# nkkrnkl/category-agnostic-pose-estimation

Hardware: AMD Instinct MI355X
Metric: episodes/sec (1-shot, 256x256, 17kpt) training step (higher is better)
Workload: dtype f32 storage/accumulate, GEMMs as bf16x3 split (3 bf16 MFMAs per product); 1 GPU; configs[1]: 1-shot training step (fwd+loss+bwd+clip+AdamW at learning rate 0, dropout on), 256x256, 17 kpt, ResNet-50 + deformable transformer, 16 episodes x 2 queries per GPU; episodes_per_gpu=16, queries_per_episode=2, image_size=256, global_batch_episodes=16, parallelism=dp1, weights=random init (no checkpoint offline)

## Files before the change

### category-agnostic-pose-estimation_amd/hip/functional.py

```python
import contextlib
import ctypes
import os

import torch

from . import lib, ops


class Runtime:
    rng = None
    direct_grad = False
    use_side_stream = os.environ.get("CAPE_SIDE_STREAM", "1") == "1"
    side = None
    on_param_grad = []
    capture_keep = None

    pending = []
    side_dirty = False

    defer_wgrad = os.environ.get("CAPE_DEFER_WGRAD", "1") == "1"
    wgrad_group = int(os.environ.get("CAPE_WGRAD_GROUP", "12"))
    wq = {}
    wq_total = 0
    wq_notify = []
    _final_cb = False

    @classmethod
    def side_stream(cls):
        if cls.side is None:
            cls.side = torch.cuda.Stream()
            cls.side_raw = cls.side.cuda_stream
        return cls.side

    @classmethod
    def join(cls):
        cls.flush_wgrads()
        if cls.side is not None and cls.side_dirty:
            cls.side_dirty = False
            lib.call("cape_stream_join", ctypes.c_void_p(ops.raw_current_stream()), ctypes.c_void_p(cls.side_raw))
            if cls.capture_keep is None:
                cls.pending.clear()

    @classmethod
    def notify(cls, *params):
        if cls.wq_total or cls.wq_notify:
            cls.wq_notify.extend(p for p in params if p is not None)
            return
        for cb in cls.on_param_grad:
            for p in params:
                if p is not None:
                    cb(p)

    @classmethod
    def enqueue_wgrad(cls, desc, keep):
        M, N, K, b_mode = desc.M, desc.N, desc.K, desc.b_mode
        key = (ops.group_tile(M, N, K), b_mode, desc.precision)
        dst = [(desc.C, desc.C + 4 * ((M - 1) * desc.ldc + N))]
        if desc.colsum_out:
            dst.append((desc.colsum_out, desc.colsum_out + 4 * M))
        items = cls.wq.setdefault(key, [])
        if any(lo < e and s < hi for it in items for s, e in it[3] for lo, hi in dst):
            cls._launch_class(key)
        cls.wq[key].append((desc, keep, (M, N, K, 1, b_mode), dst))
        cls.wq_total += 1
        if not cls._final_cb:
            try:
                torch.autograd.Variable._execution_engine.queue_callback(cls.flush_wgrads)
                cls._final_cb = True
            except RuntimeError:
                cls.flush_wgrads()
                return
        if cls.wq_total >= cls.wgrad_group or len(cls.wq[key]) >= lib.GEMM_GROUP_MAX:
            cls._flush()

    @classmethod
    def _launch_class(cls, key):
        items = cls.wq.get(key)
        if not items:
            return
        cls.wq[key] = []
        cls.wq_total -= len(items)
        tile = key[0]
        shapes = [it[2] for it in items]
        for it, sk in zip(items, ops.plan_group_splits([sh[:3] for sh in shapes], tile)):
            it[0].split_k = sk
        with _Side([t for it in items for t in it[1]]):
            for i in range(0, len(items), lib.GEMM_GROUP_MAX):
                ops.gemm_group([it[0] for it in items[i:i + lib.GEMM_GROUP_MAX]], shapes[i:i + lib.GEMM_GROUP_MAX], tile)

    @classmethod
    def flush_wgrads(cls):
        cls._final_cb = False
        cls._flush()

    @classmethod
    def _flush(cls):
        for key in list(cls.wq):
            cls._launch_class(key)
        if cls.wq_notify:
            ps, cls.wq_notify = cls.wq_notify, []
            for cb in cls.on_param_grad:
                for p in ps:
                    cb(p)

    @classmethod
    def get_rng(cls, device):
        if cls.rng is None:
            cls.rng = ops.RngState(0x5EED, device)
        return cls.rng

    @classmethod
    def seed(cls, seed, device):
        cls.rng = ops.RngState(int(seed), device)


def capturing():
    return torch.cuda.is_available() and torch.cuda.is_current_stream_capturing()


def _c(t):
    return t if (t is None or t.is_contiguous()) else t.contiguous()


class _Side:

    def __init__(self, tensors):
        self.tensors = [t for t in tensors if t is not None]

    def __enter__(self):
        self.on, self.forked, self.prev = Runtime.use_side_stream, False, ops._side[0]
        if self.on:
            Runtime.side_stream()
            ops._side[0] = self._raw
        return self

    def _raw(self):
        if not self.forked:
            self.forked = True
            lib.call("cape_stream_fork", ctypes.c_void_p(ops.raw_current_stream()), ctypes.c_void_p(Runtime.side_raw))
            Runtime.side_dirty = True
        return Runtime.side_raw

    def __exit__(self, *a):
        if not self.on:
            return False
        ops._side[0] = self.prev
        (Runtime.capture_keep if Runtime.capture_keep is not None else Runtime.pending).extend(self.tensors)
        if len(Runtime.pending) > 8192:
            Runtime.join()
        return False


def _groupable(d):
    return (d.a_mode == 1 and d.accumulate and d.b_mode in (1, 3) and d.batch == 0 and d.mask_src is None and d.bias is None
            and d.A % 16 == 0 and d.B % 16 == 0 and d.lda % 4 == 0 and d.M % 4 == 0 and d.M >= 4 and d.N % 4 == 0 and d.N >= 4
            and (d.b_mode == 3 or d.ldb % 4 == 0) and max(d.lda, d.ldb, d.ldc) < (1 << 31))


_NO_SIDE = contextlib.nullcontext()


class _ParamGrads:

    def __init__(self, refs, needs=None):
        self.refs = refs
        self.needs = [r is not None and (needs is None or bool(needs[i])) for i, r in enumerate(refs)]
        views = [self._view(r) if n else None for r, n in zip(refs, self.needs)]
# ... 1174 lines not shown
```

### category-agnostic-pose-estimation_amd/hip/lib.py

```python
import ctypes
import os

import torch

from ctypes import POINTER, c_char_p, c_float, c_int, c_int32, c_int64, c_longlong, c_size_t, c_uint32, c_uint64, c_uint8, c_void_p

_HERE = os.path.dirname(os.path.abspath(__file__))
LIB_PATH = os.environ.get("CAPE_HIP_LIB", os.path.join(_HERE, "..", "csrc", "libcape_hip.so"))
LIB_PATH = os.path.abspath(LIB_PATH)

if not os.path.exists(LIB_PATH):
    raise ImportError(
        f"libcape_hip.so not found at {LIB_PATH}; build it with `python -c 'import __graft_entry__ as g; g.build()'` "
        "(or `make -C category-agnostic-pose-estimation_amd/csrc`).  There is no CPU fallback.")
try:
    _lib = ctypes.CDLL(LIB_PATH)
except OSError as e:
    raise ImportError(f"cannot load {LIB_PATH}: {e}") from e

_lib.cape_last_error.restype = c_char_p
_lib.cape_abi_version.restype = c_int


class GemmDesc(ctypes.Structure):
# ... 7 lines not shown
        ("rng_state", c_void_p), ("rng_stream", c_uint32), ("colsum_out", c_void_p), ("precision", c_int),
        ("B_packed", c_void_p),
        ("mask_src", c_void_p), ("ldm", c_longlong), ("mask_scale", c_float),
        ("batch", c_int), ("batch_div", c_int), ("sA0", c_longlong), ("sA1", c_longlong), ("sB0", c_longlong), ("sB1", c_longlong),
        ("sC0", c_longlong), ("sC1", c_longlong),
        ("res_cols", c_int), ("sBias0", c_longlong), ("sBias1", c_longlong),
        ("cPadX", c_int), ("cKHp", c_int), ("cKWp", c_int), ("cTapH0", c_int), ("cTapHS", c_int), ("cTapW0", c_int), ("cTapWS", c_int),
    ]


class PackItem(ctypes.Structure):
    _fields_ = [("B", c_void_p), ("out", c_void_p), ("ldb", c_longlong), ("N", c_int), ("K", c_int), ("b_mode", c_int), ("pad", c_int)]


class DecodeLinearDesc(ctypes.Structure):
    _fields_ = [
        ("N", c_int), ("K", c_int), ("Nout", c_int),
        ("X", c_void_p), ("ldx", c_longlong), ("in_gamma", c_void_p), ("in_beta", c_void_p), ("in_add", c_void_p), ("ld_add", c_longlong),
        ("W", c_void_p), ("ldw", c_longlong), ("bias", c_void_p),
        ("X2", c_void_p), ("ldx2", c_longlong), ("K2", c_int), ("W2", c_void_p), ("ldw2", c_longlong), ("n2", c_int),
        ("R", c_void_p), ("ldr", c_longlong), ("res_gamma", c_void_p), ("res_beta", c_void_p),
        ("relu", c_int), ("nseg", c_int), ("seg", c_int), ("out", c_void_p * 3), ("ldo", c_longlong * 3),
    ]


class DecodeTailDesc(ctypes.Structure):
    _fields_ = [
        ("N", c_int), ("L", c_int),
        ("P4", c_void_p), ("ldp", c_longlong), ("g3", c_void_p), ("b3", c_void_p),
        ("W1", c_void_p), ("B1", c_void_p), ("W2", c_void_p), ("B2", c_void_p), ("W3", c_void_p), ("B3", c_void_p),
        ("ref", c_void_p),
        ("Wc", c_void_p), ("Bc", c_void_p), ("ncls", c_int),
        ("Wp", c_void_p), ("Bp", c_void_p), ("gp", c_void_p), ("bp", c_void_p),
        ("dim_t", c_void_p), ("vr", c_void_p),
        ("ref_out", c_void_p), ("ld_ref", c_longlong),
        ("qpos_out", c_void_p), ("refin_out", c_void_p),
        ("cls_out", c_void_p), ("ld_cls", c_longlong),
        ("hs_out", c_void_p), ("ld_hs", c_longlong),
    ]


class AugItem(ctypes.Structure):
    _fields_ = [("src", c_void_p), ("aug", c_void_p), ("out", c_void_p), ("stat", c_void_p), ("h", c_int), ("w", c_int),
                ("M", c_float * 6), ("color_on", c_int), ("order", c_int * 4),
                ("bright", c_float), ("contrast", c_float), ("sat", c_float), ("hue", c_float),
                ("mode", c_int), ("noise_std", c_float), ("seed", c_uint32), ("blur_k", c_int), ("blur_w", c_float * 49)]


DECODE_MAX_LAYERS = 8
GEMM_GROUP_MAX = 32
SUMSQ_PARTS = 256


class DecodeLayerDesc(ctypes.Structure):
    _fields_ = [(n, c_void_p) for n in (
        "w_qkv", "b_qkv", "w_qin", "k_cache", "v_cache", "w_o", "b_o", "ln2_g", "ln2_b",
        "w_sq", "b_sq", "sup_k", "sup_v", "sup_mask", "w_so", "b_so", "lns_g", "lns_b",
        "w_off", "b_off", "value", "w_mo", "b_mo", "ln1_g", "ln1_b",
        "w1", "b1", "w2", "b2", "ln3_g", "ln3_b", "m1w", "m1b", "m2w", "m2b", "m3w", "m3b")]


class DecodeStepDesc(ctypes.Structure):
    _fields_ = [
        ("N", c_int), ("n_layers", c_int), ("step", c_int), ("T", c_int), ("P", c_int), ("S", c_int), ("L", c_int),
        ("n_points", c_int), ("ncls", c_int), ("ffn_dim", c_int),
        ("shapes", c_int * 8), ("level_start", c_int * 4),
        ("emb", c_void_p), ("qpos0", c_void_p), ("refin0", c_void_p), ("ref0", c_void_p), ("vr", c_void_p), ("dim_t", c_void_p),
        ("class_w", c_void_p), ("class_b", c_void_p),
        ("pos_w", c_void_p), ("pos_b", c_void_p), ("pos_gamma", c_void_p), ("pos_beta", c_void_p),
        ("out_logits", c_void_p), ("ld_logits", c_longlong),
        ("out_coords", c_void_p), ("ld_coords", c_longlong),
        ("out_hs", c_void_p), ("ld_hs", c_longlong),
        ("layers", DecodeLayerDesc * DECODE_MAX_LAYERS),
    ]


P, I, LL, F, U32 = c_void_p, c_int, c_longlong, c_float, c_uint32
_SIGS = {
    "cape_rng_advance": [P, P],
    "cape_stream_fork": [P, P],
    "cape_stream_join": [P, P],
    "cape_gemm_f32": [POINTER(GemmDesc), P],
    "cape_gemm_group_f32": [POINTER(GemmDesc), I, I, P],
    "cape_pack_weights": [P, I, I, P],
    "cape_colsum_f32": [P, LL, I, LL, I, I, P, I, P],
    "cape_add_layernorm_fwd": [P, P, P, P, P, P, P, P, P, I, I, F, P, U32, P],
    "cape_add_layernorm_bwd": [P, P, P, P, P, P, P, P, P, P, P, I, I, F, P, U32, P],
    "cape_groupnorm_fwd": [P, P, P, P, LL, P, P, I, I, I, I, P, c_size_t, P],
    "cape_groupnorm_bwd": [P, LL, P, P, P, P, P, P, P, I, I, I, I, P, c_size_t, P],
    "cape_msda_fwd": [P, P, P, P, P, P, I, I, I, I, I, P],
    "cape_msda_bwd": [P, P, P, P, P, P, P, P, P, I, I, I, I, I, P],
    "cape_msda_bwd_ex": [P, P, P, P, P, P, P, P, P, I, I, I, I, I, I, P],
    "cape_msda_bwd_atomic": [P, P, P, P, P, P, P, P, P, I, I, I, I, I, P],
    "cape_attn_fwd": [P, P, P, P, P, LL, LL, LL, LL, LL, LL, LL, LL, I, I, I, I, F, I, I, P, F, P, U32, P],
    "cape_attn_bwd": [P, P, P, P, P, P, P, P, P, LL, LL, LL, LL, LL, LL, LL, LL, I, I, I, I, F, I, I, P, F, P, U32, P],
    "cape_flash_attn_fwd": [P, P, P, P, P, LL, LL, LL, LL, LL, LL, LL, LL, I, I, I, I, F, I, I, P, F, P, U32, P],
    "cape_flash_attn_bwd": [P, P, P, P, P, P, P, P, P, P, LL, LL, LL, LL, LL, LL, LL, LL, I, I, I, I, F, I, I, P, F, P, U32, P],
    "cape_attn_softmax_fwd": [P, P, P, I, I, I, I, F, I, I, P, F, P, U32, P],
    "cape_attn_softmax_bwd": [P, P, I, I, I, I, F, F, P, U32, P],
    "cape_add_f32": [P, P, P, LL, P],
    "cape_level_embed_add": [P, P, P, P, I, I, I, I, P],
    "cape_add_n_f32": [POINTER(c_void_p), I, P, LL, P],
    "cape_add_n_rows_f32": [POINTER(c_void_p), POINTER(c_longlong), I, P, LL, LL, I, P],
    "cape_augment_batch": [P, I, I, I, P, P, P],
    "cape_gelu_f32": [P, P, LL, P],
    "cape_support_masks": [P, P, P, I, I, I, P],
    "cape_interleave2x2_f32": [POINTER(c_void_p), P, P, I, I, I, I, P],
    "cape_gelu_bwd_f32": [P, P, P, LL, P],
    "cape_scale_residual_bwd_f32": [P, P, P, P, P, LL, I, P],
    "cape_scale_residual_f32": [P, P, P, P, LL, I, P],
    "cape_nchw_to_nhwc": [P, P, I, I, I, I, I, P],
    "cape_bn_fold": [P, P, P, P, F, P, P, I, P],
    "cape_maxpool3x3s2_nhwc": [P, P, I, I, I, I, P],
    "cape_bn_relu_bwd": [P, P, P, P, P, LL, I, I, P],
    "cape_affine_act_f32": [P, P, P, P, LL, I, I, P],
    "cape_relu_drop_bwd": [P, P, P, LL, F, P],
    "cape_pos_sine_level": [P, P, P, P, LL, I, I, I, I, P],
    "cape_token_embed_fwd": [P, P, P, P, P, P, P, P, P, P, LL, I, I, P],
    "cape_token_embed_bwd": [P, P, P, P, P, P, P, P, P, P, LL, I, I, I, P],
    "cape_query_sine_fwd": [P, P, P, LL, P],
    "cape_query_sine_bwd": [P, P, P, P, I, LL, P],
    "cape_refine_fwd": [P, P, P, LL, P],
    "cape_refine_bwd": [P, P, P, P, P, I, LL, P],
    "cape_sigmoid_fwd": [P, P, LL, P],
    "cape_sigmoid_bwd": [P, P, P, I, LL, P],
    "cape_ref_scale_fwd": [P, P, P, LL, I, I, P],
    "cape_ref_scale_bwd": [P, P, P, I, LL, I, I, P],
    "cape_support_embed_fwd": [P, P, P, P, P, P, P, I, I, I, P],
    "cape_support_embed_bwd": [P, P, P, P, P, I, I, I, P],
    "cape_adjacency": [P, P, P, P, I, I, P],
    "cape_gcn_aggregate_fwd": [P, P, P, I, I, I, P],
    "cape_gcn_aggregate_bwd": [P, P, P, P, I, I, I, P],
    "cape_zero_rows": [P, P, LL, I, P],
    "cape_legacy_coord_embed_fwd": [P, P, P, P, I, I, P],
    "cape_legacy_coord_embed_bwd": [P, P, P, P, P, P, P, I, I, P],
    "cape_support_edge_info_fwd": [P, P, P, P, LL, P, P, P, I, I, I, P],
    "cape_support_edge_info_bwd": [P, LL, P, P, P, I, I, P],
    "cape_pe_dropout_fwd": [P, P, P, I, I, I, F, P, U32, P],
    "cape_pe_dropout_bwd": [P, P, LL, F, P, U32, P],
    "cape_loss_fwd_bwd": [P, P, P, P, P, P, F, F, F, P, P, P, P, I, LL, P],
    "cape_sumsq": [P, LL, P, P],
    "cape_adamw_step": [P, P, P, P, LL, F, F, F, F, F, F, P, I, P, P, P],
    "cape_step_increment": [P, P],
    "cape_decode_next_tokens": [P, P, P, P, P, P, I, I, I, I, I, I, P],
    "cape_decode_advance": [P, LL, P, LL, P, P, P, I, I, I, I, I, I, I, P, I, I, P, P, P],
    "cape_decode_linear": [POINTER(DecodeLinearDesc), P],
    "cape_decode_tail": [POINTER(DecodeTailDesc), P],
    "cape_decode_step": [POINTER(DecodeStepDesc), P],
}
EXPORTS = ["cape_last_error", "cape_abi_version", "cape_groupnorm_workspace_bytes", "cape_packed_weight_bytes"] + list(_SIGS)
_lib.cape_packed_weight_bytes.argtypes = [I, I]
_lib.cape_packed_weight_bytes.restype = c_size_t
_lib.cape_groupnorm_workspace_bytes.argtypes = [I, I, I]
_lib.cape_groupnorm_workspace_bytes.restype = c_size_t

for _name, _args in _SIGS.items():
    _fn = getattr(_lib, _name)
    _fn.argtypes = _args
    _fn.restype = c_int


def last_error() -> str:
    return _lib.cape_last_error().decode()


def abi_version() -> int:
    return _lib.cape_abi_version()


def call(name, *args):
    rc = getattr(_lib, name)(*args)
    if rc != 0:
        raise RuntimeError(f"{name} failed: {last_error()}")


def raw():
    return _lib
```

### category-agnostic-pose-estimation_amd/hip/ops.py

```python
import ctypes
import math
import os
import weakref

import torch

from . import lib

_F32 = torch.float32


_raw_stream = getattr(torch._C, "_cuda_getCurrentRawStream", None)
_raw_device = getattr(torch._C, "_cuda_getDevice", None)


_side = [None]


def raw_current_stream():
    if _raw_stream is not None and _raw_device is not None:
        return _raw_stream(_raw_device())
    return torch.cuda.current_stream().cuda_stream


# ... 216 lines not shown
            (d.cPadX, d.cKHp, d.cKWp, d.cTapH0, d.cTapHS, d.cTapW0, d.cTapWS) = conv_sub
            assert a_mode == 3 and b_mode == 2 and _avail(B) >= d.cO * d.cKHp * d.cKWp * d.cC
            assert _avail(A) >= d.cN * d.cOH * d.cOW * d.cO and _avail(C) >= d.cN * d.cH * d.cW * d.cC
    d.scale = scale.data_ptr() if scale is not None else None
    d.bias = bias.data_ptr() if bias is not None else None
    d.residual = residual.data_ptr() if residual is not None else None
    d.ldr = ldr if ldr is not None else N
    d.res_cols = int(res_cols)
    d.relu, d.accumulate, d.split_k = int(relu), int(accumulate), int(split_k)
    d.dropout_p = float(dropout_p)
    d.rng_state = rng.t.data_ptr() if (rng is not None and dropout_p > 0) else None
    d.rng_stream = rng_stream
    d.precision = GEMM_PRECISION
    if (packed is None and PackedWeights.enabled and GEMM_PRECISION >= 1 and a_mode == 0 and b_mode in (0, 1) and batch is None
            and split_k == 1 and K in (64, 128, 256) and M > 64 and 32 <= N <= _PACK_MAX_N):
        packed = PackedWeights.lookup(B, N, K, d.ldb, b_mode)
    if packed is not None and GEMM_PRECISION >= 1:
        assert packed.dtype == torch.int16 and packed.is_cuda and packed.numel() * 2 >= lib.raw().cape_packed_weight_bytes(N, K)
        d.B_packed = packed.data_ptr()
    if mask_src is not None:
        _chk(mask_src, "gemm.mask_src")
        assert mask_src.numel() == M * N and split_k == 1
        d.mask_src, d.ldm, d.mask_scale = mask_src.data_ptr(), N, float(mask_scale)
    if colsum_out is not None:
        _chk(colsum_out, "gemm.colsum_out", contiguous=False)
        assert a_mode == 1 and _avail(colsum_out) >= M
        d.colsum_out = colsum_out.data_ptr()
    if batch is not None:
        cnt, div, sA0, sA1, sB0, sB1, sC0, sC1 = batch
        assert cnt >= 1 and div >= 1 and cnt % div == 0
        d.batch, d.batch_div = cnt, div
        d.sA0, d.sA1, d.sB0, d.sB1, d.sC0, d.sC1 = sA0, sA1, sB0, sB1, sC0, sC1
        if bias_strides is not None:
            d.sBias0, d.sBias1 = bias_strides
            assert bias is not None and _avail(bias) >= (cnt // div - 1) * d.sBias0 + (div - 1) * d.sBias1 + N
        last0, last1 = cnt // div - 1, div - 1
        offA, offB, offC = last0 * sA0 + last1 * sA1, last0 * sB0 + last1 * sB1, last0 * sC0 + last1 * sC1
    else:
        offA = offB = offC = 0
    if a_mode == 0 and M > 0:
        assert _avail(A) >= offA + (M - 1) * d.lda + K, "gemm: A too small"
    if a_mode == 1 and K > 0:
        assert _avail(A) >= offA + (K - 1) * d.lda + M, "gemm: A^T too small"
    if b_mode == 0 and N > 0:
        assert _avail(B) >= offB + (N - 1) * d.ldb + K, "gemm: B too small"
    if b_mode == 1 and K > 0:
        assert _avail(B) >= offB + (K - 1) * d.ldb + N, "gemm: B too small"
    if M > 0:
        assert _avail(C) >= offC + (M - 1) * d.ldc + N, "gemm: C too small"
    if residual is not None:
        assert res_cols % 32 == 0 and 0 <= res_cols <= N
        assert _avail(residual) >= (M - 1) * d.ldr + (res_cols or N), "gemm: residual too small"
    if bias is not None:
        assert _avail(bias) >= N
    if scale is not None:
        assert scale.numel() >= N
    return d, (A, B, C, colsum_out)


def launch_gemm(d):
    if GemmProfiler.enabled:
        e0, e1 = torch.cuda.Event(enable_timing=True), torch.cuda.Event(enable_timing=True)
        st = _stream()
        ext = torch.cuda.ExternalStream(st.value) if _side[0] is not None else None
        e0.record(ext)
        lib.call("cape_gemm_f32", ctypes.byref(d), st)
        e1.record(ext)
        M, N, K, nb = d.M, d.N, d.K, max(d.batch, 1)
        GemmProfiler.records.append((e0, e1, 2.0 * M * N * K * nb, (M, N, K, d.a_mode, d.b_mode, d.split_k, nb),
                                     GemmProfiler.alg_bytes(M, N, K, nb), 1))
        return
    lib.call("cape_gemm_f32", ctypes.byref(d), _stream())


_AUTO_SPLIT_NN = os.environ.get("CAPE_AUTO_SPLIT_NN", "1") == "1" and os.environ.get("CAPE_DETERMINISTIC", "0") != "1"
_PACK_MAX_N = int(os.environ.get("CAPE_PACK_MAX_N", "1000000"))
_GROUP_BIG_MN = int(os.environ.get("CAPE_GROUP_BIG_MN", str(64 * 1024)))


def group_tile(M, N, K):
    return 128 if (M >= 128 and N >= 128 and M * N >= _GROUP_BIG_MN and K >= 4096) else 64


def plan_group_splits(shapes, tile):
    target = 1024 if tile == 64 else 512
    tiles = [((M + tile - 1) // tile) * ((N + tile - 1) // tile) for M, N, K in shapes]
    kt = [(K + 31) // 32 for M, N, K in shapes]
    work = sum(t * k for t, k in zip(tiles, kt))
    per_block = max(8.0, work / float(target))
    out = []
    for k in kt:
        s = int(max(1, min(round(k / per_block), k // 8 if k >= 16 else 1, 64)))
        if s >= 8:
            s = s // 8 * 8
        out.append(s)
    return out


def gemm_group(descs, shapes, tile):
    n = len(descs)
    assert 1 <= n <= lib.GEMM_GROUP_MAX
    arr = (lib.GemmDesc * n)(*descs)
    if GemmProfiler.enabled:
        e0, e1 = torch.cuda.Event(enable_timing=True), torch.cuda.Event(enable_timing=True)
        st = _stream()
        ext = torch.cuda.ExternalStream(st.value) if _side[0] is not None else None
        e0.record(ext)
        lib.call("cape_gemm_group_f32", arr, n, tile, st)
        e1.record(ext)
        fl = sum(2.0 * M * N * K for M, N, K, _, _ in shapes)
        by = sum(GemmProfiler.alg_bytes(M, N, K) for M, N, K, _, _ in shapes)
        GemmProfiler.records.append((e0, e1, fl, ("group", tile, shapes[0][4], n), by, n))
        return
    lib.call("cape_gemm_group_f32", arr, n, tile, _stream())


def colsum(X, M, N, out, ldx=None, accumulate=True, nbatch=1, batch_stride=0):
    _chk(X, "colsum.X", contiguous=False)
    _chk(out, "colsum.out", contiguous=False)
    ldx = N if ldx is None else ldx
    assert M == 0 or _avail(X) >= (nbatch - 1) * batch_stride + (M - 1) * ldx + N
    assert _avail(out) >= N
    lib.call("cape_colsum_f32", _p(X), ldx, nbatch, batch_stride, M, N, _p(out), int(accumulate), _stream())


def add_layernorm_fwd(x, y, gamma, beta, pos=None, dropout_p=0.0, rng=None, rng_stream=0):
    C = x.shape[-1]
    rows = x.numel() // C
    for t, n in ((x, "x"), (y, "y"), (gamma, "gamma"), (beta, "beta"), (pos, "pos")):
        _chk(t, "ln." + n)
    if y is not None:
        assert y.shape == x.shape
    if pos is not None:
        assert pos.numel() == x.numel()
    out = torch.empty_like(x)
    mean = torch.empty(rows, dtype=_F32, device=x.device)
    rstd = torch.empty(rows, dtype=_F32, device=x.device)
    out_pos = torch.empty_like(x) if pos is not None else None
    lib.call("cape_add_layernorm_fwd", _p(x), _p(y), _p(gamma), _p(beta), _p(out), _p(mean), _p(rstd), _p(pos),
             _p(out_pos), rows, C, float(dropout_p), rng.ptr if (rng is not None and dropout_p > 0) else None,
             rng_stream, _stream())
    return out, mean, rstd, out_pos


def add_layernorm_bwd(d_out, d_out_pos, x, y, gamma, mean, rstd, dgamma, dbeta, dropout_p=0.0, rng=None, rng_stream=0):
    C = x.shape[-1]
    rows = x.numel() // C
    for t, n in ((d_out, "d_out"), (d_out_pos, "d_out_pos"), (x, "x"), (y, "y"), (dgamma, "dgamma"), (dbeta, "dbeta")):
        _chk(t, "ln_bwd." + n)
    d_x = torch.empty_like(x)
    d_y = torch.empty_like(x) if (y is not None and dropout_p > 0) else None
    lib.call("cape_add_layernorm_bwd", _p(d_out), _p(d_out_pos), _p(x), _p(y), _p(gamma), _p(mean), _p(rstd), _p(d_x),
             _p(d_y), _p(dgamma), _p(dbeta), rows, C, float(dropout_p),
             rng.ptr if (rng is not None and dropout_p > 0) else None, rng_stream, _stream())
    return d_x, (d_y if d_y is not None else d_x)


def _gn_workspace(N, C, G, device):
    nbytes = lib.raw().cape_groupnorm_workspace_bytes(N, C, G)
    return torch.empty((nbytes + 7) // 8, dtype=torch.float64, device=device), nbytes


def groupnorm_fwd(x, gamma, beta, out, out_image_stride, N, HW, C, G=32):
    for t, n in ((x, "x"), (gamma, "gamma"), (beta, "beta")):
        _chk(t, "gn." + n)
    _chk(out, "gn.out", contiguous=False)
    assert x.numel() == N * HW * C
    mean = torch.empty(N * G, dtype=_F32, device=x.device)
    rstd = torch.empty(N * G, dtype=_F32, device=x.device)
    ws, nbytes = _gn_workspace(N, C, G, x.device)
    lib.call("cape_groupnorm_fwd", _p(x), _p(gamma), _p(beta), _p(out), out_image_stride, _p(mean), _p(rstd), N, HW, C, G,
             _p(ws), nbytes, _stream())
    return mean, rstd


def groupnorm_bwd(d_out, d_out_image_stride, x, gamma, mean, rstd, dgamma, dbeta, N, HW, C, G=32):
    _chk(d_out, "gn_bwd.d_out", contiguous=False)
    d_x = torch.empty_like(x)
    ws, nbytes = _gn_workspace(N, C, G, x.device)
    lib.call("cape_groupnorm_bwd", _p(d_out), d_out_image_stride, _p(x), _p(gamma), _p(mean), _p(rstd), _p(d_x),
             _p(dgamma), _p(dbeta), N, HW, C, G, _p(ws), nbytes, _stream())
    return d_x


class LevelGeometry:

    def __init__(self, shapes):
        self.shapes = [(int(h), int(w)) for h, w in shapes]
        self.L = len(self.shapes)
        starts, s = [], 0
        for h, w in self.shapes:
            starts.append(s)
            s += h * w
        self.S = s
        self.starts = starts
        self._shapes_c = (ctypes.c_int * (2 * self.L))(*[v for hw in self.shapes for v in hw])
        self._starts_c = (ctypes.c_int * self.L)(*starts)
# ... 798 lines not shown
```

### include/cape_hip.h

```cpp
#ifndef CAPE_HIP_H
#define CAPE_HIP_H

#include <stddef.h>
#include <stdint.h>

#ifdef __cplusplus
extern "C" {
#endif

typedef void* cape_stream_t;

const char* cape_last_error(void);
int cape_abi_version(void);

int cape_rng_advance(uint64_t* rng_state, cape_stream_t stream);

int cape_stream_fork(cape_stream_t main_stream, cape_stream_t side_stream);
int cape_stream_join(cape_stream_t main_stream, cape_stream_t side_stream);

typedef struct {
  int M, N, K;
  int a_mode, b_mode;
  const float* A; long long lda;
  const float* B; long long ldb;
  float* C; long long ldc;
  int cN, cH, cW, cC, cKH, cKW, cStride, cPad, cOH, cOW, cO;
  const float* scale;
  const float* bias;
  const float* residual;
  long long ldr;
  int relu;
  int accumulate;
  int split_k;
  float dropout_p;
  const uint64_t* rng_state;
  uint32_t rng_stream;
  float* colsum_out;
  int precision;
  const uint16_t* B_packed;
  const float* mask_src; long long ldm; float mask_scale;
  int batch, batch_div; long long sA0, sA1, sB0, sB1, sC0, sC1;
  int res_cols; long long sBias0, sBias1;
  int cPadX, cKHp, cKWp, cTapH0, cTapHS, cTapW0, cTapWS;
} cape_gemm_desc;

int cape_gemm_f32(const cape_gemm_desc* d, cape_stream_t stream);

#define CAPE_GEMM_GROUP_MAX 32
int cape_gemm_group_f32(const cape_gemm_desc* descs, int n, int tile, cape_stream_t stream);

typedef struct { const float* B; uint16_t* out; long long ldb; int N, K, b_mode, pad; } cape_pack_item;
size_t cape_packed_weight_bytes(int N, int K);
int cape_pack_weights(const cape_pack_item* items_dev, int n_items, int max_blocks_per_item, cape_stream_t stream);

int cape_colsum_f32(const float* X, long long ldx, int nbatch, long long batch_stride, int M, int N, float* out,
                    int accumulate, cape_stream_t stream);

typedef struct {
  int N, K, Nout;
  const float* X; long long ldx; const float* in_gamma; const float* in_beta; const float* in_add; long long ld_add;
  const float* W; long long ldw; const float* bias;
  const float* X2; long long ldx2; int K2; const float* W2; long long ldw2; int n2;
  const float* R; long long ldr; const float* res_gamma; const float* res_beta;
  int relu;
  int nseg, seg; float* out[3]; long long ldo[3];
} cape_decode_linear_desc;
int cape_decode_linear(const cape_decode_linear_desc* d, cape_stream_t stream);

typedef struct {
  int N, L;
  const float* P4; long long ldp; const float* g3; const float* b3;
  const float* W1; const float* B1; const float* W2; const float* B2; const float* W3; const float* B3;
  const float* ref;
  const float* Wc; const float* Bc; int ncls;
  const float* Wp; const float* Bp; const float* gp; const float* bp;
  const float* dim_t; const float* vr;
  float* ref_out; long long ld_ref;
  float* qpos_out; float* refin_out;
  float* cls_out; long long ld_cls;
  float* hs_out; long long ld_hs;
} cape_decode_tail_desc;
int cape_decode_tail(const cape_decode_tail_desc* d, cape_stream_t stream);

#define CAPE_DECODE_MAX_LAYERS 8
typedef struct {
  const float *w_qkv, *b_qkv;
  const float* w_qin;
  float *k_cache, *v_cache;
  const float *w_o, *b_o, *ln2_g, *ln2_b;
  const float *w_sq, *b_sq;
  const float *sup_k, *sup_v;
  const unsigned char* sup_mask;
  const float *w_so, *b_so, *lns_g, *lns_b;
  const float *w_off, *b_off;
  const float* value;
  const float *w_mo, *b_mo, *ln1_g, *ln1_b;
  const float *w1, *b1, *w2, *b2;
  const float *ln3_g, *ln3_b;
  const float *m1w, *m1b, *m2w, *m2b, *m3w, *m3b;
} cape_decode_layer_desc;
typedef struct {
  int N, n_layers, step, T, P, S, L, n_points, ncls, ffn_dim;
  int shapes[8];
  int level_start[4];
  const float* emb;
  const float* qpos0;
  const float* refin0;
  const float* ref0;
  const float* vr;
  const float* dim_t;
  const float *class_w, *class_b;
  const float *pos_w, *pos_b, *pos_gamma, *pos_beta;
  float* out_logits; long long ld_logits;
  float* out_coords; long long ld_coords;
  float* out_hs; long long ld_hs;
  cape_decode_layer_desc layers[CAPE_DECODE_MAX_LAYERS];
} cape_decode_step_desc;
int cape_decode_step(const cape_decode_step_desc* d, cape_stream_t stream);

int cape_add_layernorm_fwd(const float* x, const float* y, const float* gamma, const float* beta,
                           float* out, float* mean, float* rstd, const float* pos, float* out_pos,
                           int rows, int C, float dropout_p, const uint64_t* rng_state, uint32_t rng_stream,
                           cape_stream_t stream);
int cape_add_layernorm_bwd(const float* d_out, const float* d_out_pos, const float* x, const float* y,
                           const float* gamma, const float* mean, const float* rstd,
                           float* d_x, float* d_y, float* dgamma, float* dbeta,
                           int rows, int C, float dropout_p, const uint64_t* rng_state, uint32_t rng_stream,
                           cape_stream_t stream);

size_t cape_groupnorm_workspace_bytes(int N, int C, int G);
int cape_groupnorm_fwd(const float* x, const float* gamma, const float* beta, float* out,
                       long long out_image_stride, float* mean, float* rstd,
                       int N, int HW, int C, int G, void* workspace, size_t workspace_bytes, cape_stream_t stream);
// ... 161 lines not shown
```

Measured before the change: 650.4 episodes/s.

## Add ordered split-K weight-gradient grouped GEMM with workspace reduction and larger tiles

Adds a dedicated grouped weight-gradient GEMM kernel with 256x128 tiles. Split-K partials are written to a workspace slab, and the last-arriving block, chosen by an atomic ticket counter, sums them in a fixed order and accumulates the result into C, with the bias colsum fused in. This replaces the previous grouped path for tile-128 dense bf16x3 and single-bf16 weight gradients. The split planner targets fewer blocks sized for the new tile. It adds a persistent workspace and counter buffer, allocated with a device sync outside capture, plus extra global traffic for the partial slabs. Reduction order becomes deterministic.

```diff
diff --git a/category-agnostic-pose-estimation_amd/csrc/gemm_wgrad.hip b/category-agnostic-pose-estimation_amd/csrc/gemm_wgrad.hip
--- /dev/null
+++ b/category-agnostic-pose-estimation_amd/csrc/gemm_wgrad.hip
@@ -0,0 +1,377 @@
+#include "gemm_common.h"
+
+namespace {
+
+constexpr int WG_MAX = CAPE_GEMM_GROUP_MAX;
+constexpr int WBM = 256, WBN = 128, WBK = 16;
+constexpr int TILE_F = WBM * WBN;
+constexpr int SLAB_F = TILE_F + WBM;
+constexpr int PLANE_B = WBK * 128 * 2;
+constexpr int BUF_B = 6 * PLANE_B;
+
+struct WgItem {
+  const float* A; const float* B; float* C; float* colsum_out;
+  float* ws; int* ctr;
+  int M, N, K, nsplit;
+  int lda, ldb, ldc, tilesN;
+  int ntiles, per, pad0, pad1;
+};
+
+struct WgArgs {
+  int n, single;
+  int bstart[WG_MAX + 1];
+  int pad;
+  WgItem it[WG_MAX];
+};
+static_assert(sizeof(WgArgs) <= 4096, "the item table travels as kernel arguments");
+
+template <bool KFULL>
+__global__ void __launch_bounds__(256, 2) gemm_wgrad_kernel(const WgArgs g) {
+  __shared__ __attribute__((aligned(16))) char lds[2 * BUF_B];
+
+  int bid = blockIdx.x;
+  int it_i = 0;
+  while (it_i + 1 < g.n && bid >= g.bstart[it_i + 1]) ++it_i;
+  const WgItem& q = g.it[it_i];
+  bid -= g.bstart[it_i];
+  const int ntiles = q.ntiles, nsplit = q.nsplit;
+  if (bid >= ntiles * nsplit) return;
+
+  int tile, split;
+  {
+    const int xcd = bid & 7, loc = bid >> 3;
+    if (nsplit > 1 && (nsplit & 7) == 0) {
+      split = xcd + 8 * (loc / ntiles);
+      tile = loc % ntiles;
+    } else if (nsplit > 1) {
+      split = bid / ntiles;
+      tile = bid - split * ntiles;
+    } else {
+      const int qq = ntiles >> 3, r = ntiles & 7;
+      tile = (xcd < r ? xcd * (qq + 1) : r * (qq + 1) + (xcd - r) * qq) + loc;
+      split = 0;
+    }
+  }
+  const int tm = tile / q.tilesN, tn = tile - tm * q.tilesN;
+  const int m0 = tm * WBM, n0 = tn * WBN;
+  const int M = q.M, N = q.N, K = q.K;
+
+  const int kb = split * q.per * BK;
+  const int ke = min(K, kb + q.per * BK);
+  const int nk = (ke - kb + WBK - 1) / WBK;
+
+  const int t = threadIdx.x;
+  const int lane = t & 63;
+  const int wave = t >> 6;
+  const int wm = wave >> 1, wn = wave & 1;
+
+  const int mc = t & 31, k0 = t >> 5;
+  const float* a_src0 = q.A + min(m0 + 4 * mc, M - 4);
+  const float* a_src1 = q.A + min(m0 + 128 + 4 * mc, M - 4);
+  const float* b_src = q.B + min(n0 + 4 * mc, N - 4);
+  const long long lda = q.lda, ldb = q.ldb;
+  const int st_off0 = tr_off<128>(2 * k0, mc >> 1) + 8 * (mc & 1);
+  const int st_off1 = tr_off<128>(2 * k0 + 1, mc >> 1) + 8 * (mc & 1);
+
+  float4 ra[2][2], rb[2];
+  auto load_tile = [&](int kt) {
+#pragma unroll
+    for (int j = 0; j < 2; ++j) {
+      const int k = kb + kt * WBK + 2 * k0 + j;
+      const bool kin = KFULL || k < K;
+      const long long kr = kin ? k : 0;
+      const float4 v0 = *reinterpret_cast<const float4*>(a_src0 + kr * lda);
+      const float4 v1 = *reinterpret_cast<const float4*>(a_src1 + kr * lda);
+      const float4 w = *reinterpret_cast<const float4*>(b_src + kr * ldb);
+      ra[0][j] = kin ? v0 : zero4();
+      ra[1][j] = kin ? v1 : zero4();
+      rb[j] = kin ? w : zero4();
+    }
+  };
+
+  const bool do_colsum = q.colsum_out != nullptr && tn == 0;
+  float4 csum[2] = {zero4(), zero4()};
+
+  auto store_tile = [&](int buf) {
+    char* base = lds + buf * BUF_B;
+    if (do_colsum) {
+#pragma unroll
+      for (int im = 0; im < 2; ++im)
+#pragma unroll
+        for (int j = 0; j < 2; ++j) { csum[im].x += ra[im][j].x; csum[im].y += ra[im][j].y; csum[im].z += ra[im][j].z; csum[im].w += ra[im][j].w; }
+    }
+#pragma unroll
+    for (int j = 0; j < 2; ++j) {
+      const int o = j ? st_off1 : st_off0;
+#pragma unroll
+      for (int im = 0; im < 2; ++im) {
+        unsigned h0, l0, h1, l1;
+        split2(ra[im][j].x, ra[im][j].y, h0, l0);
+        split2(ra[im][j].z, ra[im][j].w, h1, l1);
+        *reinterpret_cast<uint2*>(base + (2 * im) * PLANE_B + o) = make_uint2(h0, h1);
+        *reinterpret_cast<uint2*>(base + (2 * im + 1) * PLANE_B + o) = make_uint2(l0, l1);
+      }
+      unsigned h0, l0, h1, l1;
+      split2(rb[j].x, rb[j].y, h0, l0);
+      split2(rb[j].z, rb[j].w, h1, l1);
+      *reinterpret_cast<uint2*>(base + 4 * PLANE_B + o) = make_uint2(h0, h1);
+      *reinterpret_cast<uint2*>(base + 5 * PLANE_B + o) = make_uint2(l0, l1);
+    }
+  };
+
+  f32x16 acc[4][2];
+#pragma unroll
+  for (int i = 0; i < 4; ++i)
+#pragma unroll
+    for (int j = 0; j < 2; ++j)
+#pragma unroll
+      for (int r = 0; r < 16; ++r) acc[i][j][r] = 0.f;
+
+  const int tr_h = lane >> 5, tr_c = (lane >> 4) & 1, tr_q = (lane >> 2) & 3, tr_p = lane & 3;
+  const int fr_row = 8 * tr_h + tr_q, fr_chunk = 2 * tr_c + (tr_p >> 1), fr_sub = 8 * (tr_p & 1);
+  int a_fr[4], b_fr[2];
+#pragma unroll
+  for (int i = 0; i < 4; ++i) a_fr[i] = (2 * wm) * PLANE_B + tr_off<128>(fr_row, 4 * i + fr_chunk) + fr_sub;
+#pragma unroll
+  for (int j = 0; j < 2; ++j) b_fr[j] = 4 * PLANE_B + tr_off<128>(fr_row, 8 * wn + 4 * j + fr_chunk) + fr_sub;
+
+  auto compute_tile = [&](int buf) {
+    const char* base = lds + buf * BUF_B;
+    bf16x8 ahi[4], alo[4], bhi[2], blo[2];
+#pragma unroll
+    for (int i = 0; i < 4; ++i) {
+      ahi[i] = tr_read8(base + a_fr[i], 4 * 128 * 2);
+      alo[i] = tr_read8(base + a_fr[i] + PLANE_B, 4 * 128 * 2);
+    }
+#pragma unroll
+    for (int j = 0; j < 2; ++j) {
+      bhi[j] = tr_read8(base + b_fr[j], 4 * 128 * 2);
+      blo[j] = tr_read8(base + b_fr[j] + PLANE_B, 4 * 128 * 2);
+    }
+#pragma unroll
+    for (int i = 0; i < 4; ++i)
+#pragma unroll
+      for (int j = 0; j < 2; ++j) {
+        if (!g.single) {
+          acc[i][j] = __builtin_amdgcn_mfma_f32_32x32x16_bf16(alo[i], bhi[j], acc[i][j], 0, 0, 0);
+          acc[i][j] = __builtin_amdgcn_mfma_f32_32x32x16_bf16(ahi[i], blo[j], acc[i][j], 0, 0, 0);
+        }
+        acc[i][j] = __builtin_amdgcn_mfma_f32_32x32x16_bf16(ahi[i], bhi[j], acc[i][j], 0, 0, 0);
+      }
+  };
+
+  load_tile(0);
+  store_tile(0);
+  if (nk > 1) load_tile(1);
+  __syncthreads();
+  int cur = 0;
+  for (int kt = 0; kt < nk; ++kt) {
+    compute_tile(cur);
+    if (kt + 1 < nk) store_tile(cur ^ 1);
+    __syncthreads();
+    if (kt + 2 < nk) load_tile(kt + 2);
+    cur ^= 1;
+  }
+
+  float4 bias4 = zero4();
+  if (do_colsum) {
+    float4* red = reinterpret_cast<float4*>(lds);
+    red[t] = csum[0];
+    red[256 + t] = csum[1];
+    __syncthreads();
+    if (t < 64) {
+      const float4* src = red + 256 * (t >> 5) + mc;
+#pragma unroll
+      for (int i = 0; i < 8; ++i) { const float4 u = src[32 * i]; bias4.x += u.x; bias4.y += u.y; bias4.z += u.z; bias4.w += u.w; }
+    }
+    __syncthreads();
+  }
+
+  if (nsplit > 1) {
+    float* slab0 = q.ws + (long long)tile * nsplit * SLAB_F;
+    float4* mine = reinterpret_cast<float4*>(slab0 + (long long)split * SLAB_F) + wave * 2048 + lane;
+#pragma unroll
+    for (int i = 0; i < 4; ++i)
+#pragma unroll
+      for (int j = 0; j < 2; ++j)
+#pragma unroll
+        for (int r4 = 0; r4 < 4; ++r4)
+          mine[((2 * i + j) * 4 + r4) * 64] = make_float4(acc[i][j][4 * r4], acc[i][j][4 * r4 + 1], acc[i][j][4 * r4 + 2], acc[i][j][4 * r4 + 3]);
+    if (do_colsum && t < 64) *reinterpret_cast<float4*>(slab0 + (long long)split * SLAB_F + TILE_F + 4 * t) = bias4;
+    asm volatile("s_waitcnt vmcnt(0)" ::: "memory");
+    __syncthreads();
+    int* flag = reinterpret_cast<int*>(lds);
+    if (t == 0) {
+      __builtin_amdgcn_fence(__ATOMIC_RELEASE, "agent");
+      asm volatile("s_waitcnt vmcnt(0)" ::: "memory");
+      const int ticket = __hip_atomic_fetch_add(q.ctr + tile, 1, __ATOMIC_RELAXED, __HIP_MEMORY_SCOPE_AGENT);
+      const int last = ticket == nsplit - 1;
+      if (last) {
+        __builtin_amdgcn_fence(__ATOMIC_ACQUIRE, "agent");
+        asm volatile("s_waitcnt vmcnt(0)" ::: "memory");
+        __hip_atomic_store(q.ctr + tile, 0, __ATOMIC_RELAXED, __HIP_MEMORY_SCOPE_AGENT);
+      }
+      *flag = last;
+    }
+    __syncthreads();
+    if (!*flag) return;
+  }
+
+  const bool interior = (m0 + WBM <= M) && (n0 + WBN <= N);
+  const long long ldc = q.ldc;
+  auto emit = [&](int i, int j, const f32x16& v) {
+    const int ln = threadIdx.x & 63, wv = threadIdx.x >> 6;
+    const int col = n0 + (wv & 1) * 64 + j * 32 + (ln & 31);
+    const int row0 = m0 + (wv >> 1) * 128 + i * 32 + 4 * (ln >> 5);
+    float* c0 = q.C + (long long)row0 * ldc + col;
+    const bool col_ok = interior || col < N;
+    float xv[16];
+#pragma unroll
+    for (int r = 0; r < 16; ++r) {
+      const int dr = (r & 3) + 8 * (r >> 2);
+      xv[r] = (col_ok && (interior || row0 + dr < M)) ? c0[dr * ldc] : 0.f;
+    }
+#pragma unroll
+    for (int r = 0; r < 16; ++r) {
+      const int dr = (r & 3) + 8 * (r >> 2);
+      if (col_ok && (interior || row0 + dr < M)) c0[dr * ldc] = xv[r] + v[r];
+    }
+  };
+
+  if (nsplit > 1) {
+    const float* slab0 = q.ws + (long long)tile * nsplit * SLAB_F;
+    const float4* src0 = reinterpret_cast<const float4*>(slab0) + (threadIdx.x >> 6) * 2048 + (threadIdx.x & 63);
+#pragma unroll
+    for (int i = 0; i < 4; ++i) {
+      f32x16 v0, v1;
+#pragma unroll
+      for (int r = 0; r < 16; ++r) { v0[r] = 0.f; v1[r] = 0.f; }
+#pragma unroll 2
+      for (int s = 0; s < nsplit; ++s) {
+        const float4* src = src0 + (long long)s * (SLAB_F / 4) + (2 * i) * 256;
+#pragma unroll
+        for (int r4 = 0; r4 < 4; ++r4) {
+          const float4 u = src[r4 * 64], w = src[256 + r4 * 64];
+          v0[4 * r4] += u.x; v0[4 * r4 + 1] += u.y; v0[4 * r4 + 2] += u.z; v0[4 * r4 + 3] += u.w;
+          v1[4 * r4] += w.x; v1[4 * r4 + 1] += w.y; v1[4 * r4 + 2] += w.z; v1[4 * r4 + 3] += w.w;
+        }
+      }
+      emit(i, 0, v0);
+      emit(i, 1, v1);
+    }
+    if (do_colsum && t < 64) {
+      bias4 = zero4();
+      for (int s = 0; s < nsplit; ++s) {
+        const float4 u = *reinterpret_cast<const float4*>(slab0 + (long long)s * SLAB_F + TILE_F + 4 * t);
+        bias4.x += u.x; bias4.y += u.y; bias4.z += u.z; bias4.w += u.w;
+      }
+    }
+  } else {
+#pragma unroll
+    for (int i = 0; i < 4; ++i)
+#pragma unroll
+      for (int j = 0; j < 2; ++j) emit(i, j, acc[i][j]);
+  }
+  if (do_colsum && t < 64) {
+    const int m = m0 + 4 * t;
+    if (m < M) q.colsum_out[m] += bias4.x;
+    if (m + 1 < M) q.colsum_out[m + 1] += bias4.y;
+    if (m + 2 < M) q.colsum_out[m + 2] += bias4.z;
+    if (m + 3 < M) q.colsum_out[m + 3] += bias4.w;
+  }
+}
+
+struct WgPlan { size_t ws_bytes; long long counters; };
+
+inline void wg_item_geometry(const cape_gemm_desc& d, int& ntiles, int& tilesN, int& per, int& nsplit) {
+  tilesN = (d.N + WBN - 1) / WBN;
+  ntiles = ((d.M + WBM - 1) / WBM) * tilesN;
+  const int ktiles = (d.K + BK - 1) / BK;
+  const int sk = d.split_k < 1 ? 1 : d.split_k;
+  per = (ktiles + sk - 1) / sk;
+  nsplit = (ktiles + per - 1) / per;
+}
+
+int wg_validate(const char* who, const cape_gemm_desc* descs, int n, int tile, WgPlan& plan) {
+  CAPE_REQUIRE(descs != nullptr && n >= 1 && n <= WG_MAX, "%s: n=%d must be in 1..%d", who, n, WG_MAX);
+  CAPE_REQUIRE(tile == 128, "%s: the ordered k-split serves tile class 128 only", who);
+  const int prec = descs[0].precision;
+  CAPE_REQUIRE(prec == 1 || prec == 2, "%s: precision must be 1 (bf16x3) or 2 (single bf16)", who);
+  auto al16 = [](const void* p) { return (reinterpret_cast<uintptr_t>(p) & 15) == 0; };
+  plan.ws_bytes = 0;
+  plan.counters = 0;
+  for (int i = 0; i < n; ++i) {
+    const cape_gemm_desc& d = descs[i];
+    CAPE_REQUIRE(d.a_mode == 1 && d.b_mode == 1 && d.precision == prec, "%s: item %d: only dense weight gradients (a_mode 1, b_mode 1) of one precision", who, i);
+    CAPE_REQUIRE(d.M > 0 && d.N > 0 && d.K > 0 && d.A && d.B && d.C, "%s: item %d: empty product or null operand", who, i);
+    CAPE_REQUIRE(d.accumulate && !d.scale && !d.bias && !d.residual && !d.relu && d.dropout_p == 0.f && !d.mask_src && d.batch <= 1,
+                 "%s: item %d: grouped products accumulate onto C and take no other epilogue operand", who, i);
+    CAPE_REQUIRE(d.split_k >= 1, "%s: item %d: split_k must be >= 1", who, i);
+    CAPE_REQUIRE(al16(d.A) && al16(d.B) && d.lda % 4 == 0 && d.M % 4 == 0 && d.M >= 4 && d.N % 4 == 0 && d.N >= 4 && d.ldb % 4 == 0,
+                 "%s: item %d: operands must be 16-byte aligned with M, N, lda, ldb multiples of 4", who, i);
+    CAPE_REQUIRE(d.lda >= d.M && d.ldb >= d.N && d.ldc >= d.N, "%s: item %d: leading dimension shorter than the row", who, i);
+    CAPE_REQUIRE(d.lda < (1ll << 31) && d.ldb < (1ll << 31) && d.ldc < (1ll << 31), "%s: item %d: leading dimension too large", who, i);
+    int ntiles, tilesN, per, nsplit;
+    wg_item_geometry(d, ntiles, tilesN, per, nsplit);
+    if (nsplit > 1) {
+      plan.ws_bytes += (size_t)ntiles * nsplit * SLAB_F * sizeof(float);
+      plan.counters += ntiles;
+    }
+  }
+  return 0;
+}
+
+}
+
+extern "C" size_t cape_gemm_group_workspace_bytes(const cape_gemm_desc* descs, int n, int tile) {
+  WgPlan plan;
+  if (wg_validate("cape_gemm_group_workspace_bytes", descs, n, tile, plan) != 0) return (size_t)-1;
+  return plan.ws_bytes;
+}
+
+extern "C" int cape_gemm_group_ws_f32(const cape_gemm_desc* descs, int n, int tile, float* workspace, size_t workspace_bytes,
+                                      int* counters, int n_counters, cape_stream_t stream) {
+  WgPlan plan;
+  if (int rc = wg_validate("cape_gemm_group_ws_f32", descs, n, tile, plan)) return rc;
+  CAPE_REQUIRE(workspace_bytes >= plan.ws_bytes, "cape_gemm_group_ws_f32: workspace of %zu bytes, the launch needs %zu", workspace_bytes, plan.ws_bytes);
+  CAPE_REQUIRE((long long)n_counters >= plan.counters, "cape_gemm_group_ws_f32: %d arrival counters, the launch needs %lld", n_counters, plan.counters);
+  CAPE_REQUIRE(plan.ws_bytes == 0 || (workspace != nullptr && (reinterpret_cast<uintptr_t>(workspace) & 15) == 0),
+               "cape_gemm_group_ws_f32: the workspace must be 16-byte aligned");
+  CAPE_REQUIRE(plan.counters == 0 || (counters != nullptr && (reinterpret_cast<uintptr_t>(counters) & 3) == 0),
+               "cape_gemm_group_ws_f32: the counters must be 4-byte aligned");
+  WgArgs g;
+  g.n = n;
+  g.single = descs[0].precision == 2;
+  g.pad = 0;
+  bool kfull = true;
+  long long blocks = 0, ws_off = 0, ctr_off = 0;
+  for (int i = 0; i < n; ++i) {
+    const cape_gemm_desc& d = descs[i];
+    WgItem& q = g.it[i];
+    wg_item_geometry(d, q.ntiles, q.tilesN, q.per, q.nsplit);
+    q.A = d.A; q.B = d.B; q.C = d.C; q.colsum_out = d.colsum_out;
+    q.M = d.M; q.N = d.N; q.K = d.K;
+    q.lda = (int)d.lda; q.ldb = (int)d.ldb; q.ldc = (int)d.ldc;
+    q.pad0 = q.pad1 = 0;
+    q.ws = nullptr; q.ctr = nullptr;
+    if (q.nsplit > 1) {
+      q.ws = workspace + ws_off;
+      q.ctr = counters + ctr_off;
+      ws_off += (long long)q.ntiles * q.nsplit * SLAB_F;
+      ctr_off += q.ntiles;
+    }
+    kfull = kfull && (d.K % BK == 0);
+    g.bstart[i] = (int)blocks;
+    const long long nb = (long long)q.ntiles * q.nsplit;
+    blocks += (nb + 7) / 8 * 8;
+    CAPE_REQUIRE(blocks < (1ll << 30), "cape_gemm_group_ws_f32: grid too large");
+  }
+  for (int i = n; i <= WG_MAX; ++i) g.bstart[i] = (int)blocks;
+  for (int i = n; i < WG_MAX; ++i) g.it[i] = WgItem{};
+  const dim3 grid((unsigned)blocks), block(256);
+  hipStream_t s = as_stream(stream);
+  if (kfull) hipLaunchKernelGGL((gemm_wgrad_kernel<true>), grid, block, 0, s, g);
+  else hipLaunchKernelGGL((gemm_wgrad_kernel<false>), grid, block, 0, s, g);
+  CAPE_LAUNCH_CHECK("cape_gemm_group_ws_f32");
+  return 0;
+}
diff --git a/category-agnostic-pose-estimation_amd/hip/functional.py b/category-agnostic-pose-estimation_amd/hip/functional.py
--- a/category-agnostic-pose-estimation_amd/hip/functional.py
+++ b/category-agnostic-pose-estimation_amd/hip/functional.py
@@ -24,6 +24,28 @@
     wq_total = 0
     wq_notify = []
     _final_cb = False
+
+    wgrad_ws = {}
+
+    @classmethod
+    def group_workspace(cls, arr, n, tile):
+        need = lib.raw().cape_gemm_group_workspace_bytes(arr, n, tile)
+        if need == ctypes.c_size_t(-1).value:
+            raise RuntimeError(f"cape_gemm_group_workspace_bytes failed: {lib.last_error()}")
+        tiles = sum(-(-arr[i].M // ops.WGRAD_TILE_M) * -(-arr[i].N // ops.WGRAD_TILE_N) for i in range(n) if arr[i].split_k > 1)
+        dev = torch.cuda.current_device()
+        have = cls.wgrad_ws.get(dev)
+        if have is not None and have[0].numel() * 4 >= need and have[1].numel() >= tiles:
+            return have
+        if capturing():
+            return None
+        torch.cuda.synchronize(dev)
+        ws_bytes = max(need, ops._WGRAD_TARGET * 3 // 2 * ops.WGRAD_SLAB_BYTES)
+        ws = torch.empty((ws_bytes + 3) // 4, dtype=torch.float32, device=f"cuda:{dev}")
+        ctr = torch.zeros(max(tiles, 4096), dtype=torch.int32, device=f"cuda:{dev}")
+        torch.cuda.synchronize(dev)
+        cls.wgrad_ws[dev] = (ws, ctr)
+        return cls.wgrad_ws[dev]
 
     @classmethod
     def side_stream(cls):
@@ -82,7 +104,7 @@
         cls.wq_total -= len(items)
         tile = key[0]
         shapes = [it[2] for it in items]
-        for it, sk in zip(items, ops.plan_group_splits([sh[:3] for sh in shapes], tile)):
+        for it, sk in zip(items, ops.plan_group_splits([sh[:3] for sh in shapes], tile, ops.wgrad_ordered(*key))):
             it[0].split_k = sk
         with _Side([t for it in items for t in it[1]]):
             for i in range(0, len(items), lib.GEMM_GROUP_MAX):
diff --git a/category-agnostic-pose-estimation_amd/hip/lib.py b/category-agnostic-pose-estimation_amd/hip/lib.py
--- a/category-agnostic-pose-estimation_amd/hip/lib.py
+++ b/category-agnostic-pose-estimation_amd/hip/lib.py
@@ -113,6 +113,7 @@
     "cape_stream_join": [P, P],
     "cape_gemm_f32": [POINTER(GemmDesc), P],
     "cape_gemm_group_f32": [POINTER(GemmDesc), I, I, P],
+    "cape_gemm_group_ws_f32": [POINTER(GemmDesc), I, I, P, c_size_t, P, I, P],
     "cape_pack_weights": [P, I, I, P],
     "cape_colsum_f32": [P, LL, I, LL, I, I, P, I, P],
     "cape_add_layernorm_fwd": [P, P, P, P, P, P, P, P, P, I, I, F, P, U32, P],
@@ -179,7 +180,10 @@
     "cape_decode_tail": [POINTER(DecodeTailDesc), P],
     "cape_decode_step": [POINTER(DecodeStepDesc), P],
 }
-EXPORTS = ["cape_last_error", "cape_abi_version", "cape_groupnorm_workspace_bytes", "cape_packed_weight_bytes"] + list(_SIGS)
+EXPORTS = ["cape_last_error", "cape_abi_version", "cape_groupnorm_workspace_bytes", "cape_packed_weight_bytes",
+           "cape_gemm_group_workspace_bytes"] + list(_SIGS)
+_lib.cape_gemm_group_workspace_bytes.argtypes = [POINTER(GemmDesc), I, I]
+_lib.cape_gemm_group_workspace_bytes.restype = c_size_t
 _lib.cape_packed_weight_bytes.argtypes = [I, I]
 _lib.cape_packed_weight_bytes.restype = c_size_t
 _lib.cape_groupnorm_workspace_bytes.argtypes = [I, I, I]
diff --git a/category-agnostic-pose-estimation_amd/hip/ops.py b/category-agnostic-pose-estimation_amd/hip/ops.py
--- a/category-agnostic-pose-estimation_amd/hip/ops.py
+++ b/category-agnostic-pose-estimation_amd/hip/ops.py
@@ -322,9 +322,23 @@
     return 128 if (M >= 128 and N >= 128 and M * N >= _GROUP_BIG_MN and K >= 4096) else 64
 
 
-def plan_group_splits(shapes, tile):
-    target = 1024 if tile == 64 else 512
-    tiles = [((M + tile - 1) // tile) * ((N + tile - 1) // tile) for M, N, K in shapes]
+_WGRAD_ORDERED = os.environ.get("CAPE_WGRAD_ORDERED", "1") == "1"
+_WGRAD_TARGET = int(os.environ.get("CAPE_WGRAD_TARGET", "384"))
+WGRAD_TILE_M, WGRAD_TILE_N = 256, 128
+WGRAD_SLAB_BYTES = 4 * (WGRAD_TILE_M * WGRAD_TILE_N + WGRAD_TILE_M)
+
+
+def wgrad_ordered(tile, b_mode, precision):
+    return _WGRAD_ORDERED and tile == 128 and b_mode == 1 and precision in (1, 2)
+
+
+def plan_group_splits(shapes, tile, ordered=False):
+    if ordered:
+        target = _WGRAD_TARGET
+        tiles = [((M + WGRAD_TILE_M - 1) // WGRAD_TILE_M) * ((N + WGRAD_TILE_N - 1) // WGRAD_TILE_N) for M, N, K in shapes]
+    else:
+        target = 1024 if tile == 64 else 512
+        tiles = [((M + tile - 1) // tile) * ((N + tile - 1) // tile) for M, N, K in shapes]
     kt = [(K + 31) // 32 for M, N, K in shapes]
     work = sum(t * k for t, k in zip(tiles, kt))
     per_block = max(8.0, work / float(target))
@@ -341,18 +355,25 @@
     n = len(descs)
     assert 1 <= n <= lib.GEMM_GROUP_MAX
     arr = (lib.GemmDesc * n)(*descs)
+    name, extra = "cape_gemm_group_f32", ()
+    if wgrad_ordered(tile, descs[0].b_mode, descs[0].precision):
+        from . import functional
+        bufs = functional.Runtime.group_workspace(arr, n, tile)
+        if bufs is not None:
+            ws, ctr = bufs
+            name, extra = "cape_gemm_group_ws_f32", (_p(ws), ws.numel() * 4, _p(ctr), ctr.numel())
     if GemmProfiler.enabled:
         e0, e1 = torch.cuda.Event(enable_timing=True), torch.cuda.Event(enable_timing=True)
         st = _stream()
         ext = torch.cuda.ExternalStream(st.value) if _side[0] is not None else None
         e0.record(ext)
-        lib.call("cape_gemm_group_f32", arr, n, tile, st)
+        lib.call(name, arr, n, tile, *extra, st)
         e1.record(ext)
         fl = sum(2.0 * M * N * K for M, N, K, _, _ in shapes)
         by = sum(GemmProfiler.alg_bytes(M, N, K) for M, N, K, _, _ in shapes)
         GemmProfiler.records.append((e0, e1, fl, ("group", tile, shapes[0][4], n), by, n))
         return
-    lib.call("cape_gemm_group_f32", arr, n, tile, _stream())
+    lib.call(name, arr, n, tile, *extra, _stream())
 
 
 def colsum(X, M, N, out, ldx=None, accumulate=True, nbatch=1, batch_stride=0):
diff --git a/include/cape_hip.h b/include/cape_hip.h
--- a/include/cape_hip.h
+++ b/include/cape_hip.h
@@ -49,6 +49,10 @@
 #define CAPE_GEMM_GROUP_MAX 32
 int cape_gemm_group_f32(const cape_gemm_desc* descs, int n, int tile, cape_stream_t stream);
 
+size_t cape_gemm_group_workspace_bytes(const cape_gemm_desc* descs, int n, int tile);
+int cape_gemm_group_ws_f32(const cape_gemm_desc* descs, int n, int tile, float* workspace, size_t workspace_bytes,
+                           int* counters, int n_counters, cape_stream_t stream);
+
 typedef struct { const float* B; uint16_t* out; long long ldb; int N, K, b_mode, pad; } cape_pack_item;
 size_t cape_packed_weight_bytes(int N, int K);
 int cape_pack_weights(const cape_pack_item* items_dev, int n_items, int max_blocks_per_item, cape_stream_t stream);
```

After: 581.4 episodes/s. 10.6% lower.
